# araffin/srl-zoo

Hardware: AMD Instinct MI355X
Metric: images/sec (224x224x3) AE+VAE train step (higher is better)
Workload: dtype f32; 1 GPU; synthetic 224x224x3 obs, --losses autoencoder, custom_cnn, state-dim 200, bs=256 per GPU (512 frames fwd+bwd per step per GPU), Adam lr 0.005, normalised fp32 observations resident in HBM; global_batch=256, parallelism=dp1, rccl_ranks=1, devices=1

## Files before the change

### srl-zoo_amd/csrc/conv64.hip

```cpp
#include "common.h"
#include <stdlib.h>

namespace {

#ifndef SRLZ_BATCH_FWD
#define SRLZ_BATCH_FWD 16
#endif
#ifndef SRLZ_BATCH_BWD
#define SRLZ_BATCH_BWD 12
#endif
constexpr int TM = 128;
constexpr int BATCH_FWD = SRLZ_BATCH_FWD;
constexpr int NTAPS = 9;

struct ConvProg {
  int N, PH, PW, PHW, total_q;
  int G, tpg;
  long long src_gstride, dst_gstride;
  int ss, Hs, Ws;
  int ds, Hd, Wd;
  int tsrc[NTAPS], tdst[NTAPS], toff[NTAPS], tw[NTAPS];
  int tp[NTAPS + 2];
  int min_off, span;
  int s2;
// ... 133 lines not shown
  if (f.y) f.y += goff;
  if (f.dy_out) f.dy_out += goff;
  return f;
}

struct GridDiv { unsigned mPHW, mPW; int sPHW, sPW; };
__device__ __forceinline__ GridDiv grid_div(const ConvProg& P) { return GridDiv{P.mPHW, P.mPW, P.sPHW, P.sPW}; }

template <bool SWZ, int BATCH = 8, int NTHREADS = 256, bool BWD = false>
__device__ __forceinline__ void stage_rows(float* __restrict__ lds, const float* __restrict__ src, int H, int W,
                                           int stride, int cls, int PW, int PH, int total_q, int qstart,
                                           int nrows, const OpFuse f = SRLZ_NO_FUSE, int core_lo = 0, int core_n = 0,
                                           int cstride = 64, int coff = 0, const float* __restrict__ lrec = nullptr) {
  const float* __restrict__ bnp = f.bnp;
  const int t = threadIdx.x;
  const int slot = t & 15;
  const int cy = cls >> 1, cx = cls & 1;
  const int PHW = PH * PW;
  constexpr int RP = NTHREADS / 16;
  const int sn = RP / PHW, srem = RP - sn * PHW;
  const int sa = srem / PW, sb = srem - sa * PW;
  const int qq = qstart + (t >> 4) + PHW;
  int n1 = qq / PHW;
  int rem = qq - n1 * PHW;
  int a = rem / PW;
  int b = rem - a * PW;
  const int N1max = total_q / PHW;
  f32x4 sc4 = {1.f, 1.f, 1.f, 1.f}, sh4 = {0.f, 0.f, 0.f, 0.f};
  f32x4 c0 = {0.f, 0.f, 0.f, 0.f}, c1 = {0.f, 0.f, 0.f, 0.f};
  if (lrec) {
    sc4 = *(const f32x4*)(lrec + slot * 4); sh4 = *(const f32x4*)(lrec + 64 + slot * 4);
    if (BWD) { c0 = *(const f32x4*)(lrec + 128 + slot * 4); c1 = *(const f32x4*)(lrec + 192 + slot * 4); }
  } else if (bnp) { sc4 = *(const f32x4*)(bnp + 128 + slot * 4); sh4 = *(const f32x4*)(bnp + 192 + slot * 4); }
  if (!lrec && BWD && f.training) {
    const f32x4 mean = *(const f32x4*)(bnp + slot * 4), invstd = *(const f32x4*)(bnp + 64 + slot * 4);
    const f32x4 m1 = *(const f32x4*)(f.sums + slot * 4), m2 = *(const f32x4*)(f.sums + 64 + slot * 4);
#pragma unroll
    for (int e = 0; e < 4; ++e) {
      c1[e] = sc4[e] * invstd[e] * m2[e] * f.inv_count;
      c0[e] = sc4[e] * m1[e] * f.inv_count - c1[e] * mean[e];
    }
  }
  for (int base = t >> 4; base < nrows; base += RP * BATCH) {
    f32x4 v[BATCH], yv[BWD ? BATCH : 1];
    unsigned offs[BWD ? BATCH : 1];
    unsigned okmask = 0;
#pragma unroll
    for (int j = 0; j < BATCH; ++j) {
      const int y = a * stride + cy, x = b * stride + cx;
      const bool ok = base + RP * j < nrows && n1 >= 1 && n1 <= N1max && y < H && x < W;
      okmask |= (ok ? 1u : 0u) << j;
      const size_t off = (ok ? ((size_t)((n1 - 1) * H + y) * W + x) * cstride : (size_t)0) + coff + slot * 4;
      v[j] = *(const f32x4*)(src + off);
      if (BWD) { yv[j] = *(const f32x4*)(f.y + off); offs[j] = (unsigned)off; }
      b += sb; a += sa; n1 += sn;
      if (b >= PW) { b -= PW; ++a; }
      if (a >= PH) { a -= PH; ++n1; }
    }
#pragma unroll
    for (int j = 0; j < BATCH; ++j) {
      asm volatile("" : "+v"(v[j]));
      if (BWD) asm volatile("" : "+v"(yv[BWD ? j : 0]));
    }
#pragma unroll
    for (int j = 0; j < BATCH; ++j) {
      const int R = base + RP * j;
      if (R < nrows) {
        if (!((okmask >> j) & 1u)) v[j] = f32x4{0.f, 0.f, 0.f, 0.f};
        else if (bnp) {
          if (BWD) {
            const f32x4 z4 = __builtin_elementwise_fma(yv[j], sc4, sh4), t4 = __builtin_elementwise_fma(c1, yv[j], c0);
            f32x4 dz4;
#pragma unroll
            for (int e = 0; e < 4; ++e) dz4[e] = z4[e] > 0.f ? v[j][e] : 0.f;
            v[j] = __builtin_elementwise_fma(sc4, dz4, -t4);
            if (f.dy_out && (unsigned)(R - core_lo) < (unsigned)core_n) *(f32x4*)(f.dy_out + (size_t)offs[j]) = v[j];
          } else {
#pragma unroll
            for (int e = 0; e < 4; ++e) { const float z = v[j][e] * sc4[e] + sh4[e]; v[j][e] = z > 0.f ? z : 0.f; }
          }
        }
        const int sl = SWZ ? (slot ^ (R & 15)) : slot;
        *(f32x4*)(lds + R * 64 + sl * 4) = v[j];
      }
    }
  }
}

__host__ __device__ __forceinline__ int rowtab_passes(int nrows) { return ((nrows + 15) / 16 + SRLZ_BATCH_FWD - 1) / SRLZ_BATCH_FWD * SRLZ_BATCH_FWD; }

__device__ __forceinline__ void rowtab_build(unsigned* __restrict__ tab, int tpa, const ConvProg& P, int qstart, int nrows) {
  for (int R = threadIdx.x; R < 16 * tpa; R += blockDim.x) {
    unsigned e = 0;
    if (R < nrows) {
      const int qq = qstart + R + P.PHW;
      const int n1 = fastdiv(qq, P.mPHW, P.sPHW);
      const int rem = qq - n1 * P.PHW;
      const int a = fastdiv(rem, P.mPW, P.sPW);
      const int y0 = a * P.ss, x0 = (rem - a * P.PW) * P.ss;
      if ((unsigned)(n1 - 1) < (unsigned)P.N) {
        unsigned f = 0;
#pragma unroll
        for (int k = 0; k < 4; ++k) f |= (y0 + (k >> 1) < P.Hs && x0 + (k & 1) < P.Ws) ? 1u << k : 0u;
        e = ((unsigned)(((n1 - 1) * P.Hs + y0) * P.Ws + x0) << 4) | f;
      }
    }
    tab[(R & 15) * tpa + (R >> 4)] = e;
  }
}

template <int BATCH>
__device__ __forceinline__ void stage_rows_tab(float* __restrict__ lds, const float* __restrict__ src,
                                               const unsigned* __restrict__ tab, int tpa, int cls, int W, int nrows,
                                               const float* __restrict__ lrec, int cshift = 6, int coff = 0) {
  const int t = threadIdx.x;
  const int slot = t & 15, r = t >> 4;
  const unsigned delta = (unsigned)((cls >> 1) * W + (cls & 1));
  const float* __restrict__ base = src + coff + slot * 4;
  f32x4 sc4 = {1.f, 1.f, 1.f, 1.f}, sh4 = {0.f, 0.f, 0.f, 0.f};
  if (lrec) { sc4 = *(const f32x4*)(lrec + slot * 4); sh4 = *(const f32x4*)(lrec + 64 + slot * 4); }
  for (int j0 = 0; j0 < tpa; j0 += BATCH) {
    f32x4 v[BATCH];
    unsigned okmask = 0;
#pragma unroll
    for (int jj = 0; jj < BATCH; jj += 4) {
      const uint4 q = *(const uint4*)(tab + r * tpa + j0 + jj);
      const unsigned e[4] = {q.x, q.y, q.z, q.w};
#pragma unroll
      for (int i = 0; i < 4; ++i) {
        const int j = jj + i;
        const unsigned m = (unsigned)__builtin_amdgcn_sbfe((int)e[i], (unsigned)cls, 1u);
        const unsigned off = (((e[i] >> 4) + delta) << cshift) & m;
        v[j] = *(const f32x4*)(base + off);
        okmask |= m & (1u << j);
      }
    }
#pragma unroll
    for (int j = 0; j < BATCH; ++j) asm volatile("" : "+v"(v[j]));
#pragma unroll
    for (int j = 0; j < BATCH; ++j) {
      const int R = r + 16 * (j0 + j);
      if (R < nrows) {
        if (!((okmask >> j) & 1u)) v[j] = f32x4{0.f, 0.f, 0.f, 0.f};
        else if (lrec) {
#pragma unroll
          for (int e2 = 0; e2 < 4; ++e2) { const float z = v[j][e2] * sc4[e2] + sh4[e2]; v[j][e2] = z > 0.f ? z : 0.f; }
        }
        *(f32x4*)(lds + R * 64 + ((slot ^ (R & 15)) << 2)) = v[j];
      }
    }
  }
}

template <int NW, bool BWD, int PSUM>
__device__ __forceinline__ void conv64_fwd_body(const float* __restrict__ src, const float* __restrict__ wpack,
                                                const float* __restrict__ bias, float* __restrict__ dst,
                                                float* __restrict__ stats_partial, const ConvProg& P, int ntiles,
                                                const OpFuse& src_fuse_all, const PoolSum& ps) {
  static_assert(NW == 4, "8 waves of 32 x 32 measured within +-3 % in rounds 1-3 and are not kept");
  static_assert(PSUM == 0 || !BWD, "the pooled-block epilogue exists for the plain kernel");
  constexpr int NT = NW * 64;
  constexpr int NACC = 8 / NW;
  constexpr int BATCH_BWD = SRLZ_BATCH_BWD;
  extern __shared__ __attribute__((aligned(16))) unsigned char smem[];
  float* As = (float*)smem;
  float* Bs = As + (TM + P.span) * 64;
  const int tpa = rowtab_passes(TM + P.span);
  unsigned* rowtab = (unsigned*)(Bs + 4096);
  int* rowinfo = (int*)(rowtab + 16 * tpa);

  const int tid = threadIdx.x;
  const int lane = tid & 63, wave = tid >> 6;
  const int wrow = wave & 3, wcol = wave >> 2;
  const int h = lane >> 5, l31 = lane & 31;
  const int tile = xcd_remap(blockIdx.x, ntiles);
  const int grp = (P.G > 1) ? tile / P.tpg : 0;
  const int q0 = (tile - grp * P.tpg) * TM;
  src += grp * P.src_gstride;
  dst += grp * P.dst_gstride;
  const OpFuse src_fuse = fuse_for_group(src_fuse_all, grp, grp * P.src_gstride);

  if (tid < TM) {
    const int q = q0 + tid;
    int ri = -1;
    if (q < P.total_q) {
      const int n = fastdiv(q, P.mPHW, P.sPHW);
      const int rem = q - n * P.PHW;
      const int a = fastdiv(rem, P.mPW, P.sPW);
      const int ya = a * P.ds, xb = (rem - a * P.PW) * P.ds;
      if (ya < P.Hd && xb < P.Wd) ri = (((n * P.Hd + ya) * P.Wd + xb) << 2) | (ya + 1 < P.Hd ? 1 : 0) | (xb + 1 < P.Wd ? 2 : 0);
    }
    rowinfo[tid] = ri;
  }
  if constexpr (!BWD) rowtab_build(rowtab, tpa, P, q0 + P.min_off, TM + P.span);
  float* frec = (float*)(rowinfo + TM);
  if (src_fuse.bnp && tid >= NT - 64) {
    const int c = tid - (NT - 64);
    const float sc = src_fuse.bnp[128 + c], sh = src_fuse.bnp[192 + c];
    float c0 = 0.f, c1 = 0.f;
    if (BWD && src_fuse.training) {
      c1 = sc * src_fuse.bnp[64 + c] * src_fuse.sums[64 + c] * src_fuse.inv_count;
      c0 = sc * src_fuse.sums[c] * src_fuse.inv_count - c1 * src_fuse.bnp[c];
    }
    frec[c] = sc; frec[64 + c] = sh; frec[128 + c] = c0; frec[192 + c] = c1;
  }
  const float* lrec = src_fuse.bnp ? frec : nullptr;

  f32x16 acc[NACC];
  float bcol[NACC];
#pragma unroll
  for (int j = 0; j < NACC; ++j) bcol[j] = bias ? bias[(wcol * NACC + j) * 32 + l31] : 0.f;

  int cur_src = -1, cur_dst = -1;
  bool pz_new = false;

  f32x4 pA = {0.f, 0.f, 0.f, 0.f}, pB = pA, pthr = pA;
  unsigned pz_zero = 0;
  const float* __restrict__ ppool = nullptr;
  if constexpr (PSUM) {
    const float* __restrict__ rec = ps.bnp + grp * 256 + (lane & 15) * 4;
    const f32x4 mean = *(const f32x4*)rec;
    const f32x4 pinv = *(const f32x4*)(rec + 64), psh = *(const f32x4*)(rec + 192);
    const f32x4 psc = *(const f32x4*)(rec + 128);
#pragma unroll
    for (int e = 0; e < 4; ++e) {
      const bool zero = fabsf(psc[e]) <= 1e-3f * fabsf(psh[e]) || psc[e] == 0.f;
      pz_zero |= (zero ? 1u : 0u) << e;
      pthr[e] = zero ? __builtin_inff() : 0.f;
      const float isc = zero ? 0.f : 1.f / psc[e];
      pA[e] = pinv[e] * isc;
      pB[e] = -(psh[e] * isc + mean[e]) * pinv[e];
    }
    ppool = ps.pooled + grp * P.dst_gstride;
  }

  f32x4 s4 = {0.f, 0.f, 0.f, 0.f}, q4 = {0.f, 0.f, 0.f, 0.f};
  f32x4 pz[PSUM ? 8 : 1];
  auto pz_request = [&](int d) {
    const int need = d >> 1 | (d & 1) << 1;
    const unsigned ddelta = (unsigned)((d >> 1) * P.Wd + (d & 1));
#pragma unroll
    for (int hk = 0; hk < 8; ++hk) {
      const int row = wrow * 32 + 16 * (hk >> 2) + (lane >> 4) + 4 * (hk & 3);
      const int ri = rowinfo[row];
      const bool ok = ri >= 0 && (ri & need) == need;
      const unsigned pix = ok ? (unsigned)(ri >> 2) + ddelta : 0u;
      pz[PSUM ? hk : 0] = *(const f32x4*)(ppool + (size_t)pix * 64 + (lane & 15) * 4);
    }
  };
  auto flush16 = [&](int d) {
    if constexpr (PSUM == 0) {
      if (P.dbg & 2) {
        if (acc[0][0] + acc[NACC - 1][5] == 123.456f) dst[tid] = acc[0][1];
        return;
      }
    }
    const int need = d >> 1 | (d & 1) << 1;
    const unsigned ddelta = (unsigned)((d >> 1) * P.Wd + (d & 1));
    float* S = Bs + wave * 1024;
    const int eg = lane >> 4, eslot = lane & 15;
#pragma unroll
    for (int half = 0; half < 2; ++half) {
#pragma unroll
      for (int rr = 0; rr < 8; ++rr) {
        const int rowl = (rr & 3) + 8 * (rr >> 2) + 4 * h;
        const int swz = (rowl & 4) << 3;
#pragma unroll
        for (int j = 0; j < NACC; ++j) S[rowl * 64 + ((32 * j + l31) ^ swz)] = acc[j][8 * half + rr] + bcol[j];
      }
#pragma unroll
      for (int k = 0; k < 4; ++k) {
        const int rowl = eg + 4 * k;
        const int row = wrow * 32 + 16 * half + rowl;
        const f32x4 v = *(const f32x4*)(S + rowl * 64 + ((eslot ^ ((rowl & 4) << 1)) << 2));
        if constexpr (PSUM) {
          if (half == 0 && k == 0) {
#pragma unroll
            for (int hk = 0; hk < 8; ++hk) asm volatile("" : "+v"(pz[hk]));
          }
        }
        const int ri = rowinfo[row];
        const bool inside = ri >= 0 && (ri & need) == need;
        const size_t pixel = (unsigned)(ri >> 2) + ddelta;
        if (inside) {
          *(f32x4*)(dst + pixel * 64 + eslot * 4) = v;
          if constexpr (PSUM) {
            const f32x4 z = pz[half * 4 + k];
            f32x4 xh;
#pragma unroll
            for (int e = 0; e < 4; ++e) xh[e] = __builtin_fmaf(z[e], pA[e], pB[e]);
#pragma unroll
            for (int e = 0; e < 4; ++e) {
              const float dz = z[e] > pthr[e] ? v[e] : 0.f;
              s4[e] += dz; q4[e] += dz * xh[e];
            }
          } else {
#pragma unroll
            for (int e = 0; e < 4; ++e) { s4[e] += v[e]; q4[e] += v[e] * v[e]; }
          }
        }
      }
    }
    if constexpr (PSUM != 0) {
      if (pz_zero) {
        const float* __restrict__ rec = ps.bnp + grp * 256 + eslot * 4;
        const f32x4 mean = *(const f32x4*)rec, pinv = *(const f32x4*)(rec + 64), psc = *(const f32x4*)(rec + 128),
                    psh = *(const f32x4*)(rec + 192);
#pragma unroll 1
        for (int hk = 0; hk < 8; ++hk) {
          const int ri = rowinfo[wrow * 32 + 16 * (hk >> 2) + eg + 4 * (hk & 3)];
          if (!(ri >= 0 && (ri & need) == need)) continue;
          const size_t pixel = (unsigned)(ri >> 2) + ddelta;
          const int n = (int)pixel / (P.Hd * P.Wd);
          const int y = ((int)pixel - n * P.Hd * P.Wd) / P.Wd, x = (int)pixel - (n * P.Hd + y) * P.Wd;
          const uint32_t packed = *(const uint32_t*)(ps.argmax + (size_t)grp * P.dst_gstride + pixel * 64 + eslot * 4);
          const f32x4 v = *(const f32x4*)(dst + pixel * 64 + eslot * 4);
#pragma unroll
          for (int e = 0; e < 4; ++e)
            if ((pz_zero >> e) & 1u) {
              const int a = (packed >> (8 * e)) & 0xff;
              const int iy = y * 2 - ps.pad + a / 3, ix = x * 2 - ps.pad + a % 3;
              const float vy = ps.y[grp * ps.y_gstride + ((size_t)(n * ps.H + iy) * ps.W + ix) * 64 + eslot * 4 + e];
              const float dz = vy * psc[e] + psh[e] > 0.f ? v[e] : 0.f;
              s4[e] += dz; q4[e] += dz * ((vy - mean[e]) * pinv[e]);
            }
        }
      }
    }
  };

  constexpr int BV = 1024 / NT;
  const int bslot = wave * (BV * 64) + lane;
  f32x4 breg[BV];
  {
    const f32x4* wsrc = (const f32x4*)(wpack + (size_t)P.tw[0] * 4096);
#pragma unroll
    for (int i = 0; i < BV; ++i) breg[i] = wsrc[bslot + i * 64];
  }
  int w0 = P.tp[0], w1 = P.tp[1];
  if constexpr (PSUM == 1) {
    __syncthreads();
    pz_request(P.tdst[0]);
  }
  constexpr int TAP_UNROLL = BWD ? NTAPS : 3;
#pragma unroll TAP_UNROLL
  for (int ti = 0; ti < NTAPS; ++ti) {
    const int w2 = P.tp[ti + 2];
    const int tsrc = (w0 >> 20) & 3, tdst = (w0 >> 22) & 3;
    __syncthreads();
    if (tdst != cur_dst) {
      if (cur_dst >= 0) flush16(cur_dst);
#pragma unroll
      for (int j = 0; j < NACC; ++j)
#pragma unroll
        for (int r = 0; r < 16; ++r) acc[j][r] = 0.f;
      if constexpr (PSUM == 2) pz_new = true;
      cur_dst = tdst;
    }
    if (tsrc != cur_src) {
      if (!(P.dbg & 1)) {
        if (BWD)
          stage_rows<true, (NW == 4 ? BATCH_BWD : 2), NT, true>(As, src, P.Hs, P.Ws, P.ss, tsrc, P.PW, P.PH, P.total_q,
                                                        q0 + P.min_off, TM + P.span, src_fuse, -P.min_off, TM, 64, 0, lrec);
        else
          stage_rows_tab<BATCH_FWD>(As, src, rowtab, tpa, tsrc, P.Ws, TM + P.span, lrec);
      }
      cur_src = tsrc;
    }
    {
      f32x4* wdst = (f32x4*)Bs;
#pragma unroll
      for (int i = 0; i < BV; ++i) wdst[bslot + i * 64] = breg[i];
    }
    if constexpr (PSUM == 2) {
      if (pz_new) { pz_request(cur_dst); pz_new = false; }
    }
    __syncthreads();
    if (BWD ? ti + 1 < NTAPS : true) {
      const f32x4* wsrc = (const f32x4*)(wpack + (size_t)((w1 >> 16) & 15) * 4096);
#pragma unroll
      for (int i = 0; i < BV; ++i) breg[i] = wsrc[bslot + i * 64];
    }
    __builtin_amdgcn_sched_barrier(0);
    const int R = wrow * 32 + l31 + (int)(short)(w0 & 0xffff) - P.min_off;
    int abase = (R * 64 + ((h ^ (R & 15)) << 2)) * 4;
    asm volatile("" : "+v"(abase));
    const float* brow = Bs + (wcol * NACC * 32 + l31) * 64;
    const int bkey = lane & 15;
    f32x4 a = *(const f32x4*)((const char*)As + abase);
    f32x4 b[NACC];
#pragma unroll
    for (int j = 0; j < NACC; ++j) b[j] = *(const f32x4*)(brow + j * 2048 + ((h ^ bkey) << 2));
#pragma unroll
    for (int kc = 0; kc < 8; ++kc) {
      f32x4 an = a, bn[NACC];
#pragma unroll
      for (int j = 0; j < NACC; ++j) bn[j] = b[j];
      if (kc < 7) {
        const int slot = (kc + 1) * 2 + h;
        an = *(const f32x4*)((const char*)As + (abase ^ ((kc + 1) << 5)));
#pragma unroll
        for (int j = 0; j < NACC; ++j) bn[j] = *(const f32x4*)(brow + j * 2048 + ((slot ^ bkey) << 2));
      }
      __builtin_amdgcn_sched_barrier(0);
#pragma unroll
      for (int r = 0; r < 4; ++r)
#pragma unroll
        for (int j = 0; j < NACC; ++j) acc[j] = __builtin_amdgcn_mfma_f32_32x32x2f32(a[r], b[j][r], acc[j], 0, 0, 0);
      a = an;
#pragma unroll
      for (int j = 0; j < NACC; ++j) b[j] = bn[j];
    }
    w0 = w1; w1 = w2;
  }
  __syncthreads();
  flush16(cur_dst);

  if (stats_partial && !(P.dbg & 2)) {
    __syncthreads();
    float* red = Bs;
#pragma unroll
    for (int e = 0; e < 4; ++e) {
      s4[e] += __shfl_xor(s4[e], 16, 64); s4[e] += __shfl_xor(s4[e], 32, 64);
      q4[e] += __shfl_xor(q4[e], 16, 64); q4[e] += __shfl_xor(q4[e], 32, 64);
    }
    if (lane < 16) {
      *(f32x4*)(red + wrow * 128 + lane * 4) = s4;
      *(f32x4*)(red + wrow * 128 + 64 + lane * 4) = q4;
    }
    __syncthreads();
    if (tid < 128) {
      const float v = red[tid] + red[128 + tid] + red[256 + tid] + red[384 + tid];
      stats_partial[(size_t)tile * 128 + tid] = v;
    }
  }
}

template <int NW, bool BWD = false>
__global__ __launch_bounds__(NW * 64, NW / 2) void conv64_fwd_kernel(const float* __restrict__ src,
                                                                    const float* __restrict__ wpack,
                                                                    const float* __restrict__ bias,
                                                                    float* __restrict__ dst,
                                                                    float* __restrict__ stats_partial,
                                                                    const ConvProg P, int ntiles, const OpFuse src_fuse_all) {
  conv64_fwd_body<NW, BWD, 0>(src, wpack, bias, dst, stats_partial, P, ntiles, src_fuse_all, SRLZ_NO_POOLSUM);
}

template <int PSUM>
__global__ __launch_bounds__(256, 2) void conv64_dgrad_poolsum_kernel(const float* __restrict__ src,
                                                                     const float* __restrict__ wpack,
                                                                     float* __restrict__ dst,
                                                                     float* __restrict__ bn_bwd_partial, const ConvProg P,
                                                                     int ntiles, const PoolSum ps) {
  conv64_fwd_body<4, false, PSUM>(src, wpack, nullptr, dst, bn_bwd_partial, P, ntiles, SRLZ_NO_FUSE, ps);
}

constexpr int GP_THREADS = 512;
constexpr int GP_RP = GP_THREADS / 16;
constexpr int GP_BATCH = 6;
constexpr int GP_CORE = TM / GP_RP;

struct GatherRows {
  f32x4 v[GP_BATCH], yv[GP_BATCH];
  unsigned offs[GP_CORE];
  unsigned ok;
};

constexpr int GT_P = 8;
constexpr int GT_WORDS = GP_RP * GT_P;
__device__ __forceinline__ void gtab_build(unsigned* __restrict__ tab, const ConvProg& P, int q0, int nrows) {
  int R = threadIdx.x;
  asm volatile("" : "+v"(R));
  if (R < GT_WORDS) {
    unsigned e = 0;
    if (R < nrows) {
      const int qq = q0 + R;
      const int n = fastdiv(qq, P.mPHW, P.sPHW);
      const int rem = qq - n * P.PHW;
      const int a = fastdiv(rem, P.mPW, P.sPW);
      const int y0 = 2 * a, x0 = 2 * (rem - a * P.PW);
      if (n < P.N) {
        unsigned f = 0;
#pragma unroll
        for (int k = 0; k < 4; ++k) f |= (y0 + (k >> 1) < P.Hs && x0 + (k & 1) < P.Ws) ? 1u << k : 0u;
        e = ((unsigned)((n * P.Hs + y0) * P.Ws + x0) << 4) | f;
      }
    }
    tab[(R & (GP_RP - 1)) * GT_P + (R >> 5)] = e;
  }
}

template <int NJ = GP_BATCH>
__device__ __forceinline__ void gather_request(GatherRows& r, const float* __restrict__ src, const float* __restrict__ y,
                                               const unsigned* __restrict__ tab, int cls, int W) {
  int t = threadIdx.x;
  asm volatile("" : "+v"(t));
  const int slot = t & 15;
  const unsigned delta = (unsigned)((cls >> 1) * W + (cls & 1));
  const unsigned* __restrict__ tp = tab + (t >> 4) * GT_P;
  const uint4 e03 = *(const uint4*)tp;
  uint2 e45 = {0u, 0u};
  if constexpr (NJ > 4) e45 = *(const uint2*)(tp + 4);
  const unsigned e[GP_BATCH] = {e03.x, e03.y, e03.z, e03.w, e45.x, e45.y};
  static_assert(GP_BATCH == 6 && NJ >= GP_CORE && NJ <= GP_BATCH, "the table read above takes six rows");
  unsigned okmask = 0;
#pragma unroll
  for (int j = 0; j < NJ; ++j) {
    const unsigned m = (unsigned)__builtin_amdgcn_sbfe((int)e[j], (unsigned)cls, 1u);
    const unsigned off = ((((e[j] >> 4) + delta) << 6) & m) + slot * 4;
    r.v[j] = *(const f32x4*)(src + off);
    r.yv[j] = *(const f32x4*)(y + off);
    if (j < GP_CORE) r.offs[j] = off;
    okmask |= m & (1u << j);
  }
  r.ok = okmask;
}

__device__ __forceinline__ __amdgpu_buffer_rsrc_t gp_buffer(float* p, unsigned bytes) {
  return __builtin_amdgcn_make_buffer_rsrc(p, 0, (int)bytes, 0x00020000);
}
constexpr unsigned GP_DROP = 0xFFFFFF00u;

struct PlainRows {
  f32x4 v[GP_BATCH];
  unsigned ok;
};

__device__ __forceinline__ void gtab_build_shifted(unsigned* __restrict__ tab, const ConvProg& P, int qstart, int nrows) {
  int R = threadIdx.x;
  asm volatile("" : "+v"(R));
  if (R < GT_WORDS) {
    unsigned e = 0;
    if (R < nrows) {
      const int qq = qstart + R + P.PHW;
      const int n1 = fastdiv(qq, P.mPHW, P.sPHW);
      const int rem = qq - n1 * P.PHW;
      const int a = fastdiv(rem, P.mPW, P.sPW);
      const int y0 = 2 * a, x0 = 2 * (rem - a * P.PW);
      if ((unsigned)(n1 - 1) < (unsigned)P.N) {
        unsigned f = 0;
#pragma unroll
        for (int k = 0; k < 4; ++k) f |= (y0 + (k >> 1) < P.Hs && x0 + (k & 1) < P.Ws) ? 1u << k : 0u;
        e = ((unsigned)(((n1 - 1) * P.Hs + y0) * P.Ws + x0) << 4) | f;
      }
    }
    tab[(R & (GP_RP - 1)) * GT_P + (R >> 5)] = e;
  }
}

__device__ __forceinline__ void plain_request(PlainRows& r, const float* __restrict__ src, const unsigned* __restrict__ tab, int cls,
                                              int W) {
  int t = threadIdx.x;
  asm volatile("" : "+v"(t));
  const int slot = t & 15;
  const unsigned delta = (unsigned)((cls >> 1) * W + (cls & 1));
  const unsigned* __restrict__ tp = tab + (t >> 4) * GT_P;
  const uint4 e03 = *(const uint4*)tp;
  const uint2 e45 = *(const uint2*)(tp + 4);
  const unsigned e[GP_BATCH] = {e03.x, e03.y, e03.z, e03.w, e45.x, e45.y};
  unsigned okmask = 0;
#pragma unroll
  for (int j = 0; j < GP_BATCH; ++j) {
    const unsigned m = (unsigned)__builtin_amdgcn_sbfe((int)e[j], (unsigned)cls, 1u);
    const unsigned off = ((((e[j] >> 4) + delta) << 6) & m) + slot * 4;
    r.v[j] = *(const f32x4*)(src + off);
    okmask |= m & (1u << j);
  }
  r.ok = okmask;
}

__device__ __forceinline__ void plain_land(float* __restrict__ lds, PlainRows& r, int nrows) {
  int t = threadIdx.x;
  asm volatile("" : "+v"(t));
  const int slot = t & 15;
#pragma unroll
  for (int j = 0; j < GP_BATCH; ++j) {
    const int R = (t >> 4) + GP_RP * j;
    const f32x4 v = ((r.ok >> j) & 1u) ? r.v[j] : f32x4{0.f, 0.f, 0.f, 0.f};
    if (R < nrows) *(f32x4*)(lds + R * 64 + ((slot ^ (R & 15)) << 2)) = v;
  }
}

__global__ __launch_bounds__(GP_THREADS, 4) void conv64_gather_pipe_kernel(const float* __restrict__ src_all,
                                                                          const float* __restrict__ wpack,
                                                                          float* __restrict__ dst_all,
                                                                          float* __restrict__ stats_partial, const ConvProg P,
                                                                          int ntiles) {
  extern __shared__ __attribute__((aligned(16))) unsigned char smem[];
  float* As = (float*)smem;
  float* Bs = As + (TM + P.span) * 64;
  int* rowinfo = (int*)(Bs + 4096);
  unsigned* gtab = (unsigned*)(rowinfo + 6 * TM);
  float* red = (float*)(gtab + GT_WORDS);

  const int tid = threadIdx.x;
  const int lane = tid & 63, wave = tid >> 6;
  const int nrows = TM + P.span;
  const int cls0 = P.tsrc[0], cls1 = P.tsrc[4], cls2 = P.tsrc[6], cls3 = P.tsrc[8];

  const int xcd = blockIdx.x & 7, wi = blockIdx.x >> 3, wpx = gridDim.x >> 3;
  const int tq = ntiles >> 3, tr = ntiles & 7;
  const int tbase = (xcd < tr) ? xcd * (tq + 1) : tr * (tq + 1) + (xcd - tr) * tq;
  const int tcnt = tq + (xcd < tr ? 1 : 0);

  constexpr int BV = 1024 / GP_THREADS;
  const int bslot = wave * (BV * 64) + lane;
  f32x4 breg[BV];
  {
    const f32x4* wsrc = (const f32x4*)(wpack + (size_t)P.tw[0] * 4096);
#pragma unroll
    for (int i = 0; i < BV; ++i) breg[i] = wsrc[bslot + i * 64];
  }
  const unsigned dst_bytes = (unsigned)P.dst_gstride * 4u;

  PlainRows rr;
  int k = wi;
  int parity = 0;
  if (k < tcnt) {
    const int tile = tbase + k;
    const int grp = (P.G > 1 && tile >= P.tpg) ? 1 : 0;
    const int q0 = (tile - grp * P.tpg) * TM;
    gtab_build_shifted(gtab, P, q0 + P.min_off, nrows);
    __syncthreads();
    plain_request(rr, src_all + grp * P.src_gstride, gtab, cls0, P.Ws);
    plain_land(As, rr, nrows);
  }
  for (; k < tcnt; k += wpx, parity ^= 1) {
    const int tile = tbase + k;
    const int grp = (P.G > 1 && tile >= P.tpg) ? 1 : 0;
    const int q0 = (tile - grp * P.tpg) * TM;
    const float* __restrict__ src = src_all + grp * P.src_gstride;
    const __amdgpu_buffer_rsrc_t dst = gp_buffer(dst_all + grp * P.dst_gstride, dst_bytes);
    const int k2 = k + wpx;
    const int tile2 = tbase + (k2 < tcnt ? k2 : k);
    const int grp2 = (P.G > 1 && tile2 >= P.tpg) ? 1 : 0;
    const int q02 = (tile2 - grp2 * P.tpg) * TM;
    int* ri = rowinfo + parity * (3 * TM);
    if (tid < TM) {
      const int q = q0 + tid;
      int n = -1, ya = 0, xb = 0;
      if (q < P.total_q) {
        n = fastdiv(q, P.mPHW, P.sPHW);
        const int rem = q - n * P.PHW;
        const int a = fastdiv(rem, P.mPW, P.sPW);
        ya = a * P.ds;
        xb = (rem - a * P.PW) * P.ds;
      }
      ri[tid] = n; ri[TM + tid] = ya; ri[2 * TM + tid] = xb;
    }
    f32x16 acc;
#pragma unroll
    for (int r = 0; r < 16; ++r) acc[r] = 0.f;
    int tid_t = tid;
    asm volatile("" : "+v"(tid_t));
    const int lane_t = tid_t & 63, wave_t = tid_t >> 6;
    const int wrow_t = wave_t & 3, wcol_t = wave_t >> 2;
    const int h_t = lane_t >> 5, l31_t = lane_t & 31;
    const int arow0 = wrow_t * 32 + l31_t - P.min_off;
    const float* brow = Bs + (wcol_t * 32 + l31_t) * 64;
    const int bkey = lane_t & 15;
    const int bslot_t = wave_t * (BV * 64) + lane_t;

#pragma unroll
    for (int ti = 0; ti < NTAPS; ++ti) {
      __syncthreads();
      {
        f32x4* wdst = (f32x4*)Bs;
#pragma unroll
        for (int i = 0; i < BV; ++i) wdst[bslot_t + i * 64] = breg[i];
      }
      {
        const f32x4* wsrc = (const f32x4*)(wpack + (size_t)P.tw[(ti + 1) % NTAPS] * 4096);
#pragma unroll
        for (int i = 0; i < BV; ++i) breg[i] = wsrc[bslot_t + i * 64];
// ... 1063 lines not shown
      int go = b * (8 * 64);
      asm volatile("" : "+v"(go));
      float bf[4][4];
#pragma unroll
      for (int c = 0; c < 4; ++c)
#pragma unroll
        for (int i = 0; i < 4; ++i) bf[c][i] = gcol[c * TK * 64 + go + 2 * i * 64];
#pragma unroll
      for (int t = 0; t < NTAPS; ++t) {
        const float* ap = scol + u[t] * 64;
        float af[4];
#pragma unroll
        for (int i = 0; i < 4; ++i) af[i] = ap[2 * i * 64];
#pragma unroll
        for (int i = 0; i < 4; ++i) acc[t] = __builtin_amdgcn_mfma_f32_32x32x2f32(af[i], bf[GRP[t]][i], acc[t], 0, 0, 0);
        u[t] += 8;
        if (u[t] >= RING_ROWS_S2) u[t] -= RING_ROWS_S2;
      }
    }
    __syncthreads();
    if (more) {
      g_land();
      rows64_store<true, 0, 2, RING_ROWS_S2>(Ss, q0 + P.min_off + TK + P.span, ps, oks, xq);
    }
    __syncthreads();
  }
  float* out = partial + (size_t)blockIdx.x * (NTAPS * 4096);
#pragma unroll
  for (int t = 0; t < NTAPS; ++t) {
    float* o = out + (size_t)P.tw[t] * 4096;
#pragma unroll
    for (int r = 0; r < 16; ++r) {
      const int row = mi * 32 + (r & 3) + 8 * (r >> 2) + 4 * h;
      o[row * 64 + nj * 32 + l31] = acc[t][r];
    }
  }
  __syncthreads();
  float* red = Ss;
  *(f32x4*)(red + (tid >> 4) * 64 + (tid & 15) * 4) = bs4;
  __syncthreads();
  if (tid < 64) {
    float* bout = partial + (size_t)gridDim.x * (NTAPS * 4096) + (size_t)blockIdx.x * 64;
    float t = 0.f;
#pragma unroll
    for (int r = 0; r < 16; ++r) t += red[r * 64 + tid];
    bout[tid] = t;
  }
}

__global__ __launch_bounds__(1024) void conv64_wgrad_reduce(const float* __restrict__ partial, int nwg,
                                                           float* __restrict__ dw_ref, float* __restrict__ dbias,
                                                           int transposed, int interleaved) {
  const int o = threadIdx.x & 255, part = threadIdx.x >> 8;
  const int id = blockIdx.x * 256 + o;
  constexpr int TOT = NTAPS * 4096;
  const int per = (nwg + 3) / 4;
  const int w0 = part * per, w1 = (w0 + per < nwg) ? w0 + per : nwg;
  double s0 = 0.0, s1 = 0.0, s2 = 0.0, s3 = 0.0;
  if (id < TOT + 64) {
    const float* base = interleaved ? partial + id : (id < TOT) ? partial + id : partial + (size_t)nwg * TOT + (id - TOT);
    const size_t stride = interleaved ? (size_t)interleaved : (id < TOT) ? (size_t)TOT : 64;
    int w = w0;
    for (; w + 3 < w1; w += 4) {
      s0 += (double)base[(size_t)w * stride];
      s1 += (double)base[(size_t)(w + 1) * stride];
      s2 += (double)base[(size_t)(w + 2) * stride];
      s3 += (double)base[(size_t)(w + 3) * stride];
    }
    for (; w < w1; ++w) s0 += (double)base[(size_t)w * stride];
  }
  __shared__ double sm[4][256];
  sm[part][o] = (s0 + s1) + (s2 + s3);
  __syncthreads();
  if (part == 0 && id < TOT + 64) {
    const double s = (sm[0][o] + sm[1][o]) + (sm[2][o] + sm[3][o]);
    if (id < TOT) {
      const int tap = id >> 12, ci = (id >> 6) & 63, co = id & 63;
      dw_ref[transposed ? ((ci * 64 + co) * 9 + tap) : ((co * 64 + ci) * 9 + tap)] = (float)s;
    } else if (dbias) {
      dbias[id - TOT] = (float)s;
    }
  }
}

__global__ void conv64_pack_kernel(const float* __restrict__ w_ref, float* __restrict__ pf, float* __restrict__ pb,
                                   int transposed) {
  const int id = blockIdx.x * blockDim.x + threadIdx.x;
  if (id >= NTAPS * 4096) return;
  const int tap = id >> 12, n = (id >> 6) & 63, k = id & 63;
  const int o = (tap * 64 + n) * 64 + ((((k >> 2) ^ (n & 15)) << 2) | (k & 3));
  const int fwd_idx = transposed ? ((k * 64 + n) * 9 + tap) : ((n * 64 + k) * 9 + tap);
  const int bwd_idx = transposed ? ((n * 64 + k) * 9 + tap) : ((k * 64 + n) * 9 + tap);
  if (pf) pf[o] = w_ref[fwd_idx];
  if (pb) pb[o] = w_ref[bwd_idx];
}

static int check_desc(const srlz_conv64_desc* d) {
  SRLZ_REQUIRE(d != nullptr, SRLZ_ERR_NULL, "conv64: null descriptor");
  SRLZ_REQUIRE(d->ksize == 3 && (d->stride == 1 || d->stride == 2) && d->n > 0, SRLZ_ERR_BAD_DESC,
               "conv64: only 3x3 stride 1/2 supported (k=%d s=%d)", d->ksize, d->stride);
  SRLZ_REQUIRE(d->groups >= 0 && (d->groups <= 1 || d->n % d->groups == 0), SRLZ_ERR_BAD_DESC,
               "conv64: n = %d is not a multiple of groups = %d", d->n, d->groups);
  int eho, ewo;
  if (!d->transposed) {
    eho = (d->hi + 2 * d->pad - 3) / d->stride + 1;
    ewo = (d->wi + 2 * d->pad - 3) / d->stride + 1;
  } else {
    eho = (d->hi - 1) * d->stride - 2 * d->pad + 3;
    ewo = (d->wi - 1) * d->stride - 2 * d->pad + 3;
  }
  SRLZ_REQUIRE(eho == d->ho && ewo == d->wo, SRLZ_ERR_BAD_DESC, "conv64: output size %dx%d inconsistent (expected %dx%d)",
               d->ho, d->wo, eho, ewo);
  return 0;
}

static int program_for(ConvProg* P, const srlz_conv64_desc* d, int backward_data) {
  int rc;
  const int G = d->groups > 1 ? d->groups : 1;
  if (!backward_data)
    rc = build_program(P, !d->transposed, d->stride, d->pad, d->n, d->hi, d->wi, d->ho, d->wo, G);
  else
    rc = build_program(P, d->transposed, d->stride, d->pad, d->n, d->ho, d->wo, d->hi, d->wi, G);
  SRLZ_REQUIRE(rc == 0, SRLZ_ERR_BAD_DESC, "conv64: cannot build a grid program for this descriptor");
  return 0;
}

static size_t fwd_lds_bytes(const ConvProg& P) {
  return (size_t)(TM + P.span) * 256 + 16384 + (size_t)64 * rowtab_passes(TM + P.span) + TM * 4 + 256 * 4;
}
static size_t convn_lds_bytes(const ConvProg& P) {
  return (size_t)(TM + P.span) * 256 + 16384 + (size_t)64 * rowtab_passes(TM + P.span) + TM * 4 + 8 * 128 * 4;
}
static size_t wgrad_lds_bytes(const ConvProg& P, int tk) { return (size_t)(tk + P.span + tk) * 256; }
static int wgrad_tk(const ConvProg& P) { (void)P; return 64; }

constexpr int GATHER_PIPE_MIN_TILES_PER_GROUP = 256;
static bool gather_pipe_ok(const ConvProg& P) {
  if (P.tpg < GATHER_PIPE_MIN_TILES_PER_GROUP) return false;
  bool grouped = P.s2 && P.ss == 2 && P.G <= 2 && !P.dbg;
  for (int t = 0; t < NTAPS; ++t) grouped = grouped && P.tsrc[t] == P.tsrc[t < 4 ? 0 : t < 6 ? 4 : t < 8 ? 6 : 8] && P.tdst[t] == 0;
  const bool fits32 = P.src_gstride * 4 < (1LL << 32) - 65536 && P.dst_gstride * 4 < (1LL << 32) - 65536;
  return grouped && fits32 && TM + P.span <= GP_RP * GP_BATCH && GP_RP <= P.PHW && -P.min_off <= P.PHW;
}

static int launch_fwd(const float* src, const float* wpack, const float* bias, float* dst, float* stats,
                      const ConvProg& P, hipStream_t st, const OpFuse src_fuse = SRLZ_NO_FUSE, const PoolSum* psum = nullptr) {
  const int ntiles = P.G * P.tpg;
  const size_t lds = fwd_lds_bytes(P);
  SRLZ_REQUIRE(lds <= 160 * 1024, SRLZ_ERR_BAD_DESC, "conv64: tile needs %zu bytes of LDS", lds);
  SRLZ_REQUIRE((long long)P.N * P.Hs * P.Ws * 64 < (1LL << 32) && (long long)P.N * P.Hd * P.Wd < (1LL << 29) &&
                   (long long)P.total_q + P.PHW + TM + P.span < (1LL << 31),
               SRLZ_ERR_BAD_DESC, "conv64: a group of %d images of %d x %d -> %d x %d is beyond the tile tables' 32-bit offsets", P.N, P.Hs,
               P.Ws, P.Hd, P.Wd);
  if (psum) {
    SRLZ_REQUIRE(!src_fuse.y && !src_fuse.bnp && stats && !bias, SRLZ_ERR_BAD_DESC, "conv64: the pooled-block epilogue takes a plain operand");
    bool one_class = true;
    for (int t = 1; t < NTAPS; ++t) one_class = one_class && P.tdst[t] == P.tdst[0];
    if (one_class) {
      SRLZ_MAX_LDS(conv64_dgrad_poolsum_kernel<1>, lds);
      SRLZ_LAUNCH(conv64_dgrad_poolsum_kernel<1>, dim3(ntiles), dim3(256), lds, st, src, wpack, dst, stats, P, ntiles, *psum);
    } else {
      SRLZ_MAX_LDS(conv64_dgrad_poolsum_kernel<2>, lds);
      SRLZ_LAUNCH(conv64_dgrad_poolsum_kernel<2>, dim3(ntiles), dim3(256), lds, st, src, wpack, dst, stats, P, ntiles, *psum);
    }
    return 0;
  }
#define SRLZ_FWD_LAUNCH(NWV, BWDV)                                                                                          \
  do {                                                                                                                     \
    SRLZ_MAX_LDS((conv64_fwd_kernel<NWV, BWDV>), lds);                                                                      \
    SRLZ_LAUNCH((conv64_fwd_kernel<NWV, BWDV>), dim3(ntiles), dim3(NWV * 64), lds, st, src, wpack, bias, dst, stats,        \
                P, ntiles, src_fuse);                                                                                      \
  } while (0)
  if (src_fuse.y) {
    SRLZ_REQUIRE((long long)P.N * P.Hs * P.Ws * 64 < (1LL << 32), SRLZ_ERR_BAD_DESC,
                 "conv64: a group's operand has %lld floats (the fused staging keeps 32-bit row offsets)", (long long)P.N * P.Hs * P.Ws * 64);
    SRLZ_FWD_LAUNCH(4, true);
  } else {
    if (!src_fuse.bnp && !bias && gather_pipe_ok(P)) {
      int pgrid = 2 * srlz_device_cus();
      if (pgrid > ntiles) pgrid = ntiles;
      pgrid &= ~7;
      if (pgrid < 8) pgrid = 8;
      const size_t plds = (size_t)(TM + P.span) * 256 + 16384 + 6 * TM * 4 + GT_WORDS * 4 + 8 * 64 * 4;
      SRLZ_MAX_LDS(conv64_gather_pipe_kernel, plds);
      SRLZ_LAUNCH(conv64_gather_pipe_kernel, dim3(pgrid), dim3(GP_THREADS), plds, st, src, wpack, dst, stats, P, ntiles);
      return 0;
    }
    SRLZ_FWD_LAUNCH(4, false);
  }
#undef SRLZ_FWD_LAUNCH
  return 0;
}

static int make_bwd_fuse(OpFuse* f, const srlz_bn_bwd_operand* o, const char* who) {
  *f = SRLZ_NO_FUSE;
  if (!o) return 0;
  SRLZ_REQUIRE(o->y && o->bnp && o->sums && o->count > 0, SRLZ_ERR_NULL, "%s: incomplete srlz_bn_bwd_operand", who);
  f->bnp = o->bnp; f->y = o->y; f->sums = o->sums; f->training = o->training;
  f->inv_count = 1.0f / (float)(double)o->count;
  f->dy_out = o->dy_out;
  return 0;
}

static bool wgrad_gather_ok(const ConvProg& P) {
  bool grouped = P.s2 && P.ss == 2 && !P.dbg;
  for (int t = 0; t < NTAPS; ++t) grouped = grouped && P.tsrc[t] == P.tsrc[t < 4 ? 0 : t < 6 ? 4 : t < 8 ? 6 : 8] && P.tdst[t] == 0;
  return grouped && WG_TK + P.span <= 16 * WG_SROWS && (long long)P.N * P.Hs * P.Ws * 64 < (1LL << 32) &&
         (long long)P.N * P.Hd * P.Wd * 64 < (1LL << 32) && (long long)P.total_q + P.PHW + WG_TK + P.span < (1LL << 31);
}

static int wgrad_grid(const ConvProg& P) {
  const int tk = wgrad_tk(P);
  const int nchunks = (P.total_q + tk - 1) / tk;
  int g = 2 * srlz_device_cus() / P.G;
  if (g > nchunks) g = nchunks;
  if (g < 1) g = 1;
  return g * P.G;
}


__global__ __launch_bounds__(256, 2) void convN_fwd_kernel(const float* __restrict__ src, const float* __restrict__ wpack,
                                                          float* __restrict__ dst, float* __restrict__ stats_partial,
                                                          const ConvProg P, int ntiles, int nci, int nco,
                                                          const float* __restrict__ src_bnp, int only_tap, int cshift) {
  constexpr int NT = 256;
  extern __shared__ __attribute__((aligned(16))) unsigned char smem[];
  float* As = (float*)smem;
  float* Bs = As + (TM + P.span) * 64;
  const int tpa = rowtab_passes(TM + P.span);
  unsigned* rowtab = (unsigned*)(Bs + 4096);
  int* rowinfo = (int*)(rowtab + 16 * tpa);
  float* frec = (float*)(rowinfo + TM);

  const int tid = threadIdx.x;
  const int lane = tid & 63, wave = tid >> 6;
  const int h = lane >> 5, l31 = lane & 31;
  const int tile = xcd_remap(blockIdx.x, ntiles);
  const int co = blockIdx.y;
  const int cout = nco * 64;
  const int grp = (P.G > 1) ? tile / P.tpg : 0;
  const int q0 = (tile - grp * P.tpg) * TM;
  src += (size_t)grp * P.src_gstride * nci;
  dst += (size_t)grp * P.dst_gstride * nco;
  if (src_bnp) src_bnp += (size_t)grp * nci * 256;

  if (tid < TM) {
    const int q = q0 + tid;
    int ri = -1;
    if (q < P.total_q) {
      const int n = fastdiv(q, P.mPHW, P.sPHW);
      const int rem = q - n * P.PHW;
      const int a = fastdiv(rem, P.mPW, P.sPW);
      const int ya = a * P.ds, xb = (rem - a * P.PW) * P.ds;
      if (ya < P.Hd && xb < P.Wd) ri = (n * P.Hd + ya) * P.Wd + xb;
    }
    rowinfo[tid] = ri;
  }
  rowtab_build(rowtab, tpa, P, q0 + P.min_off, TM + P.span);
  if (src_bnp)
    for (int i = tid; i < nci * 128; i += NT) frec[i] = src_bnp[(i >> 7) * 256 + 128 + (i & 127)];

  f32x16 acc[2];
#pragma unroll
  for (int j = 0; j < 2; ++j)
#pragma unroll
    for (int r = 0; r < 16; ++r) acc[j][r] = 0.f;

  constexpr int BV = 1024 / NT;
  const int bslot = wave * (BV * 64) + lane;
  f32x4 breg[BV];
  const float* wbase = wpack + (size_t)co * nci * NTAPS * 4096;
  const int t_first = only_tap >= 0 ? only_tap : 0, t_count = only_tap >= 0 ? 1 : NTAPS;
  {
    const f32x4* wsrc = (const f32x4*)(wbase + (size_t)P.tw[t_first] * 4096);
#pragma unroll
    for (int i = 0; i < BV; ++i) breg[i] = wsrc[bslot + i * 64];
  }
  const int nsteps = nci * t_count;
  int ci = 0, tk = 0;
  int cur_src = -1;
  for (int step = 0; step < nsteps; ++step) {
    const int ti = t_first + tk;
    const int tsrc = P.tsrc[ti], toff = P.toff[ti];
    int tk2 = tk + 1, ci2 = ci;
    if (tk2 == t_count) { tk2 = 0; ci2 = ci + 1; }
    __syncthreads();
    if (tk == 0 || tsrc != cur_src) {
      stage_rows_tab<BATCH_FWD>(As, src, rowtab, tpa, tsrc, P.Ws, TM + P.span, src_bnp ? frec + ci * 128 : nullptr, cshift, ci * 64);
      cur_src = tsrc;
    }
    {
      f32x4* wdst = (f32x4*)Bs;
#pragma unroll
      for (int i = 0; i < BV; ++i) wdst[bslot + i * 64] = breg[i];
    }
    __syncthreads();
    {
      const int cn = ci2 < nci ? ci2 : 0;
      const f32x4* wsrc = (const f32x4*)(wbase + ((size_t)cn * NTAPS + P.tw[t_first + tk2]) * 4096);
#pragma unroll
      for (int i = 0; i < BV; ++i) breg[i] = wsrc[bslot + i * 64];
    }
    __builtin_amdgcn_sched_barrier(0);
    const int R = wave * 32 + l31 + toff - P.min_off;
    int abase = (R * 64 + ((h ^ (R & 15)) << 2)) * 4;
    asm volatile("" : "+v"(abase));
// ... 377 lines not shown
```

Measured before the change: 44900 images/s.

## Use buffer stores with pre-decoded row offsets and fold accumulator zeroing into MFMA

In the plain forward conv kernel, row info is re-encoded as tile-relative byte offsets plus flags. Each wave decodes it into registers once, and the epilogue writes through a raw buffer store whose out-of-range offset drops masked rows, so per-row branches and 64-bit address math go away. The explicit zeroing of the accumulators at each new output class is replaced by a first MFMA with a zero C operand, selected by a scalar branch in inline asm. The change adds register pressure and a new 32-bit offset limit, enforced by a host-side check.

```diff
diff --git a/srl-zoo_amd/csrc/conv64.hip b/srl-zoo_amd/csrc/conv64.hip
--- a/srl-zoo_amd/csrc/conv64.hip
+++ b/srl-zoo_amd/csrc/conv64.hip
@@ -309,6 +309,28 @@
   }
 }
 
+__device__ __forceinline__ __amdgpu_buffer_rsrc_t gp_buffer(float* p, unsigned bytes) {
+  return __builtin_amdgcn_make_buffer_rsrc(p, 0, (int)bytes, 0x00020000);
+}
+constexpr unsigned GP_DROP = 0xFFFFFF00u;
+__device__ __forceinline__ void mfma_first2(f32x16& acc0, f32x16& acc1, float a, float b0, float b1, int open) {
+  asm volatile(
+      "s_nop 1\n\t"
+      "s_cmp_lg_u32 %5, 0\n\t"
+      "s_cbranch_scc1 1f\n\t"
+      "v_mfma_f32_32x32x2_f32 %0, %2, %3, %0\n\t"
+      "v_mfma_f32_32x32x2_f32 %1, %2, %4, %1\n\t"
+      "s_branch 2f\n"
+      "1:\n\t"
+      "v_mfma_f32_32x32x2_f32 %0, %2, %3, 0\n\t"
+      "v_mfma_f32_32x32x2_f32 %1, %2, %4, 0\n"
+      "2:"
+      : "+v"(acc0), "+v"(acc1)
+      : "v"(a), "v"(b0), "v"(b1), "s"(open)
+      : "scc");
+}
+constexpr unsigned FWD_DROP = 0xC0000000u;
+
 template <int NW, bool BWD, int PSUM>
 __device__ __forceinline__ void conv64_fwd_body(const float* __restrict__ src, const float* __restrict__ wpack,
                                                 const float* __restrict__ bias, float* __restrict__ dst,
@@ -336,6 +358,7 @@
   src += grp * P.src_gstride;
   dst += grp * P.dst_gstride;
   const OpFuse src_fuse = fuse_for_group(src_fuse_all, grp, grp * P.src_gstride);
+  const int pixbase = fastdiv(q0, P.mPHW, P.sPHW) * (P.Hd * P.Wd);
 
   if (tid < TM) {
     const int q = q0 + tid;
@@ -347,6 +370,7 @@
       const int ya = a * P.ds, xb = (rem - a * P.PW) * P.ds;
       if (ya < P.Hd && xb < P.Wd) ri = (((n * P.Hd + ya) * P.Wd + xb) << 2) | (ya + 1 < P.Hd ? 1 : 0) | (xb + 1 < P.Wd ? 2 : 0);
     }
+    if constexpr (PSUM == 0 && !BWD) ri = ri < 0 ? 0 : (int)(((unsigned)((ri >> 2) - pixbase) << 8) | (unsigned)(ri & 3) | 4u);
     rowinfo[tid] = ri;
   }
   if constexpr (!BWD) rowtab_build(rowtab, tpa, P, q0 + P.min_off, TM + P.span);
@@ -393,6 +417,17 @@
 
   f32x4 s4 = {0.f, 0.f, 0.f, 0.f}, q4 = {0.f, 0.f, 0.f, 0.f};
   f32x4 pz[PSUM ? 8 : 1];
+  constexpr bool DEC = PSUM == 0 && !BWD;
+  unsigned roff[DEC ? 8 : 1], rflags = 0;
+  const long long left = (P.dst_gstride - (long long)pixbase * 64) * 4;
+  auto decode_rows = [&]() {
+#pragma unroll
+    for (int hk = 0; hk < 8; ++hk) {
+      const unsigned ri = (unsigned)rowinfo[wrow * 32 + 16 * (hk >> 2) + (lane >> 4) + 4 * (hk & 3)];
+      roff[DEC ? hk : 0] = (ri & ~255u) | ((unsigned)(lane & 15) * 16u);
+      rflags |= (ri & 7u) << (3 * hk);
+    }
+  };
   auto pz_request = [&](int d) {
     const int need = d >> 1 | (d & 1) << 1;
     const unsigned ddelta = (unsigned)((d >> 1) * P.Wd + (d & 1));
@@ -416,6 +451,9 @@
     const unsigned ddelta = (unsigned)((d >> 1) * P.Wd + (d & 1));
     float* S = Bs + wave * 1024;
     const int eg = lane >> 4, eslot = lane & 15;
+    const long long cleft = left - (long long)ddelta * 256;
+    const __amdgpu_buffer_rsrc_t dbuf =
+        gp_buffer(dst + (size_t)(pixbase + (int)ddelta) * 64, cleft < (long long)FWD_DROP - 256 ? (unsigned)cleft : FWD_DROP - 256u);
 #pragma unroll
     for (int half = 0; half < 2; ++half) {
 #pragma unroll
@@ -430,6 +468,17 @@
         const int rowl = eg + 4 * k;
         const int row = wrow * 32 + 16 * half + rowl;
         const f32x4 v = *(const f32x4*)(S + rowl * 64 + ((eslot ^ ((rowl & 4) << 1)) << 2));
+        if constexpr (DEC) {
+          const unsigned m = (unsigned)(need | 4) << (3 * (half * 4 + k));
+          const bool inside = (rflags & m) == m;
+          unsigned voff = inside ? roff[DEC ? half * 4 + k : 0] : FWD_DROP;
+          asm volatile("" : "+v"(voff));
+          __builtin_amdgcn_raw_buffer_store_b128(v, dbuf, voff, 0, 0);
+          const f32x4 vv = inside ? v : f32x4{0.f, 0.f, 0.f, 0.f};
+          s4 += vv;
+          q4 = __builtin_elementwise_fma(vv, vv, q4);
+          continue;
+        }
         if constexpr (PSUM) {
           if (half == 0 && k == 0) {
 #pragma unroll
@@ -505,12 +554,10 @@
     const int w2 = P.tp[ti + 2];
     const int tsrc = (w0 >> 20) & 3, tdst = (w0 >> 22) & 3;
     __syncthreads();
-    if (tdst != cur_dst) {
+    const bool open = tdst != cur_dst;
+    if (open) {
       if (cur_dst >= 0) flush16(cur_dst);
-#pragma unroll
-      for (int j = 0; j < NACC; ++j)
-#pragma unroll
-        for (int r = 0; r < 16; ++r) acc[j][r] = 0.f;
+      else if constexpr (DEC) decode_rows();
       if constexpr (PSUM == 2) pz_new = true;
       cur_dst = tdst;
     }
@@ -560,8 +607,9 @@
         for (int j = 0; j < NACC; ++j) bn[j] = *(const f32x4*)(brow + j * 2048 + ((slot ^ bkey) << 2));
       }
       __builtin_amdgcn_sched_barrier(0);
-#pragma unroll
-      for (int r = 0; r < 4; ++r)
+      if (kc == 0) mfma_first2(acc[0], acc[NACC - 1], a[0], b[0][0], b[NACC - 1][0], __builtin_amdgcn_readfirstlane(open ? 1 : 0));
+#pragma unroll
+      for (int r = (kc == 0 ? 1 : 0); r < 4; ++r)
 #pragma unroll
         for (int j = 0; j < NACC; ++j) acc[j] = __builtin_amdgcn_mfma_f32_32x32x2f32(a[r], b[j][r], acc[j], 0, 0, 0);
       a = an;
@@ -672,11 +720,6 @@
   }
   r.ok = okmask;
 }
-
-__device__ __forceinline__ __amdgpu_buffer_rsrc_t gp_buffer(float* p, unsigned bytes) {
-  return __builtin_amdgcn_make_buffer_rsrc(p, 0, (int)bytes, 0x00020000);
-}
-constexpr unsigned GP_DROP = 0xFFFFFF00u;
 
 struct PlainRows {
   f32x4 v[GP_BATCH];
@@ -2046,6 +2089,8 @@
                    (long long)P.total_q + P.PHW + TM + P.span < (1LL << 31),
                SRLZ_ERR_BAD_DESC, "conv64: a group of %d images of %d x %d -> %d x %d is beyond the tile tables' 32-bit offsets", P.N, P.Hs,
                P.Ws, P.Hd, P.Wd);
+  SRLZ_REQUIRE(psum || src_fuse.y || (127LL / P.PHW + 2) * P.Hd * P.Wd < (1LL << 23), SRLZ_ERR_BAD_DESC,
+               "conv64: a tile's %lld images of %d x %d are beyond the flush's 32-bit byte offsets", 127LL / P.PHW + 2, P.Hd, P.Wd);
   if (psum) {
     SRLZ_REQUIRE(!src_fuse.y && !src_fuse.bnp && stats && !bias, SRLZ_ERR_BAD_DESC, "conv64: the pooled-block epilogue takes a plain operand");
     bool one_class = true;
```

After: 45120 images/s (median of 6 runs). Within noise of the previous version (+0.5%).
